# vressegu/sdeflow-light

Hardware: AMD Instinct MI355X
Metric: score-matching train steps/sec (+ reverse-SDE sample steps/sec) (higher is better)
Workload: dtype f32

## Files before the change

sdeflow_light_amd/csrc/conv_kernels.hip:

```cpp
#include "common.h"
#include <type_traits>
#include <stdlib.h>

#define CONV_MAX_SRC 2

__device__ __forceinline__ f32x4 mfma16c(float a, float b, f32x4 c) {
  return __builtin_amdgcn_mfma_f32_16x16x4f32(a, b, c, 0, 0, 0);
}

struct ConvGeom {
  int N, Hi, Wi, Ho, Wo;
  int KH, KW, strideH, padH, strideW, padW;
  int mode;
  int ups;
};

struct ConvArgs {
  ConvGeom g;
  const float* src[CONV_MAX_SRC];
  int C[CONV_MAX_SRC];
  int koff[CONV_MAX_SRC];
  int nsrc;
  const float* Wp;
  int Cout, CoutP, Ktot;
  const float* bias;
  const float* samp_bias;
  int n_bias, n_samp;
  float* out;
  int accumulate;
  const float* residual;
  const float* in_scale;
  const float* in_shift;
  int in_act;
  unsigned short tapmask_in[16];
  unsigned short tapmask_out[8];
  float* cstat;
  int cs_S;
};

__device__ __forceinline__ float row16_sum(float v) {
  v += __builtin_bit_cast(float, __builtin_amdgcn_update_dpp(0, __builtin_bit_cast(int, v), 0xB1, 0xF, 0xF, false));
  v += __builtin_bit_cast(float, __builtin_amdgcn_update_dpp(0, __builtin_bit_cast(int, v), 0x4E, 0xF, 0xF, false));
  v += __builtin_bit_cast(float, __builtin_amdgcn_update_dpp(0, __builtin_bit_cast(int, v), 0x141, 0xF, 0xF, false));
  v += __builtin_bit_cast(float, __builtin_amdgcn_update_dpp(0, __builtin_bit_cast(int, v), 0x140, 0xF, 0xF, false));
  return v;
}
__device__ __forceinline__ void cstat_store(const ConvArgs& A, int n, int slot, int co, f32x4 s, f32x4 ss, int il) {
#pragma unroll
  for (int r = 0; r < 4; ++r) { s[r] = row16_sum(s[r]); ss[r] = row16_sum(ss[r]); }
  if (il == 0) {
    float* cp = A.cstat + (((size_t)n * A.cs_S + slot) * 2) * A.Cout + co;
    *reinterpret_cast<f32x4*>(cp) = s;
    *reinterpret_cast<f32x4*>(cp + A.Cout) = ss;
  }
}


__device__ __forceinline__ bool src_coord(const ConvGeom& g, int o, int k, int in_size_up, int stride, int pad, int& i) {
  int v;
  if (g.mode == 0) {
    v = o * stride + k - pad;
  } else {
    const int t = o + pad - k;
    if (t < 0) return false;
    if (stride == 2) { if (t & 1) return false; v = t >> 1; }
    else if (stride == 1) v = t;
    else { if (t % stride) return false; v = t / stride; }
  }
  if (v < 0 || v >= in_size_up) return false;
  i = g.ups ? (v >> 1) : v;
  return true;
}

template <int MT, int NT, bool FAST>
__global__ void __launch_bounds__(256) k_conv_gemm(ConvArgs A) {
  const int tid = threadIdx.x, w = tid >> 6, lane = tid & 63, il = lane & 15, q = lane >> 4;
  const ConvGeom g = A.g;
  const int HoWo = g.Ho * g.Wo;
  const int Mtot = g.N * HoWo;
  const int m0 = (blockIdx.x * 4 + w) * (NT * 16);
  if (m0 >= Mtot) return;
  const int co0 = blockIdx.y * (MT * 16);
  const int Hup = g.ups ? 2 * g.Hi : g.Hi, Wup = g.ups ? 2 * g.Wi : g.Wi;
// ... 712 lines not shown
        valid |= 1u << k;
      }
    }
    st[k] = v;
  }
#pragma unroll
  for (int k = 0; k < NST; ++k) {
    const int idx = tid + 256 * k;
    if (idx < n_items) {
      f32x4 v = st[k];
      if (A.in_scale && ((valid >> k) & 1u)) {
        v = v * ga + gb;
        if (A.in_act == 1) {
#pragma unroll
          for (int r = 0; r < 4; ++r) v[r] = v[r] * __builtin_amdgcn_rcpf(1.0f + __expf(-v[r]));
        }
      }
      *reinterpret_cast<f32x4*>(cs_lds + (idx >> 3) * CT_P + 4 * c4) = v;
    }
  }
  __syncthreads();
  const int py = tid >> 4, px = tid & 15;
  float acc[CO];
#pragma unroll
  for (int co = 0; co < CO; ++co) acc[co] = 0.f;
#pragma unroll
  for (int tap = 0; tap < 9; ++tap) {
    const float* xp = cs_lds + ((py + tap / 3) * HW + px + tap % 3) * CT_P;
    const float* wt = A.Wp + (size_t)tap * A.CoutP * A.Ktot;
#pragma unroll
    for (int q4 = 0; q4 < 8; ++q4) {
      const f32x4 xv = *reinterpret_cast<const f32x4*>(xp + 4 * q4);
#pragma unroll
      for (int co = 0; co < CO; ++co) {
        const float* w = wt + (size_t)co * A.Ktot + 4 * q4;
        acc[co] = __builtin_fmaf(xv[0], w[0], acc[co]); acc[co] = __builtin_fmaf(xv[1], w[1], acc[co]);
        acc[co] = __builtin_fmaf(xv[2], w[2], acc[co]); acc[co] = __builtin_fmaf(xv[3], w[3], acc[co]);
      }
    }
#pragma unroll
    for (int co = 0; co < CO; ++co) asm volatile("" : "+v"(acc[co]));
  }
  const int oy = y0 + py, ox = x0 + px;
  if (oy < g.Ho && ox < g.Wo) {
    const size_t m = ((size_t)n * g.Ho + oy) * g.Wo + ox;
    float* op = A.out + m * CO;
#pragma unroll
    for (int co = 0; co < CO; ++co) {
      float v = acc[co];
      if (n < A.n_bias && A.bias) v += A.bias[co];
      if (A.samp_bias && n < A.n_samp) v += A.samp_bias[(size_t)n * CO + co];
      if (A.accumulate) v += op[co];
      if (A.residual) v += A.residual[m * CO + co];
      op[co] = v;
    }
  }
}

__device__ __forceinline__ float dpp_from_next_lane(float v) {
  return __builtin_bit_cast(float, __builtin_amdgcn_update_dpp(0, __builtin_bit_cast(int, v), 0x101 , 0xf, 0xf, true));
}
template <int HW_>
__device__ __forceinline__ void wino_patch_load(f32x4 (&d)[4][4], const float* __restrict__ p00, bool last_in_row) {
#pragma unroll
  for (int i = 0; i < 4; ++i) {
    d[i][0] = *reinterpret_cast<const f32x4*>(p00 + (i * HW_ + 0) * CT_P);
    d[i][1] = *reinterpret_cast<const f32x4*>(p00 + (i * HW_ + 1) * CT_P);
  }
#pragma unroll
  for (int i = 0; i < 4; ++i)
#pragma unroll
    for (int j = 0; j < 2; ++j)
#pragma unroll
      for (int r = 0; r < 4; ++r) d[i][2 + j][r] = dpp_from_next_lane(d[i][j][r]);
  if (last_in_row) {
#pragma unroll
    for (int i = 0; i < 4; ++i) {
      d[i][2] = *reinterpret_cast<const f32x4*>(p00 + (i * HW_ + 2) * CT_P);
      d[i][3] = *reinterpret_cast<const f32x4*>(p00 + (i * HW_ + 3) * CT_P);
    }
  }
}

template <int NCO, bool WL = false>
__global__ void __launch_bounds__(256, 2) k_conv_wino(ConvArgs A, int tiles_x, int tiles_y, int n_tiles, int n_cob, int n_tgrp) {
  extern __shared__ __attribute__((aligned(16))) float cw_lds[];
  const int tid = threadIdx.x, w = tid >> 6, lane = tid & 63, il = lane & 15, q = lane >> 4;
  const ConvGeom g = A.g;
  constexpr int HW = 18, halo = 18 * 18;
  float* cur = cw_lds;
  const int xcd = blockIdx.x & 7, loc = blockIdx.x >> 3;
  const int cob = loc % n_cob, tile = (loc / n_cob) * 8 + xcd;
  (void)n_tgrp;
  if (tile >= n_tiles) return;
  const int co0 = cob * (NCO * 16);
  const int tt = 16 * w + il, ty = tt >> 3, tx = tt & 7;
  const int pbase = (2 * ty * HW + 2 * tx) * CT_P + 4 * q;
  f32x4 acc[16][NCO];
#pragma unroll
  for (int p = 0; p < 16; ++p)
#pragma unroll
    for (int c = 0; c < NCO; ++c) acc[p][c] = f32x4{0, 0, 0, 0};

  int nch[CONV_MAX_SRC];
#pragma unroll
  for (int s = 0; s < CONV_MAX_SRC; ++s) nch[s] = s < A.nsrc ? (A.C[s] + CT_KC - 1) / CT_KC : 0;
  constexpr int MAXST = (halo * (CT_KC / 4) + 255) / 256;
  constexpr int n_items = halo * (CT_KC / 4);
  const int up = g.ups ? 1 : 0;
  const int ctot_all = A.C[0] + (A.nsrc > 1 ? A.C[1] : 0);
  int n, y0, x0;
  { int t = tile; const int tx_i = t % tiles_x; t /= tiles_x; const int ty_i = t % tiles_y; n = t / tiles_y; y0 = ty_i * 16; x0 = tx_i * 16; }
  auto stage = [&](int s_, int c0) __attribute__((always_inline)) {
    const int C = A.C[s_];
    const float* base = A.src[s_] + (size_t)n * g.Hi * g.Wi * C;
    f32x4 ga = {1.f, 1.f, 1.f, 1.f}, gb = {0.f, 0.f, 0.f, 0.f};
    const int cq = c0 + 4 * (tid & 7);
    if (A.in_scale && cq < C) {
      const size_t o = (size_t)n * ctot_all + (s_ ? A.C[0] : 0) + cq;
      ga = *reinterpret_cast<const f32x4*>(A.in_scale + o);
      gb = *reinterpret_cast<const f32x4*>(A.in_shift + o);
    }
    f32x4 st[MAXST];
    unsigned valid = 0;
#pragma unroll
    for (int k = 0; k < MAXST; ++k) {
      const int idx = tid + 256 * k;
      f32x4 v = {0, 0, 0, 0};
      if (idx < n_items) {
        const int hp = idx >> 3, hy = hp / HW, hx = hp - hy * HW;
        const int iy = y0 + hy - 1, ix = x0 + hx - 1;
        const int c = c0 + 4 * (idx & 7);
        if (iy >= 0 && iy < (g.Hi << up) && ix >= 0 && ix < (g.Wi << up) && c < C) {
          v = *reinterpret_cast<const f32x4*>(base + ((size_t)(iy >> up) * g.Wi + (ix >> up)) * C + c);
          valid |= 1u << k;
        }
      }
      st[k] = v;
    }
    if (A.in_scale) {
#pragma unroll
      for (int k = 0; k < MAXST; ++k) {
        if ((valid >> k) & 1u) {
          f32x4 v = st[k] * ga + gb;
          if (A.in_act == 1) {
#pragma unroll
            for (int r = 0; r < 4; ++r) v[r] = v[r] * __builtin_amdgcn_rcpf(1.0f + __expf(-v[r]));
          }
          st[k] = v;
        }
      }
    }
#pragma unroll
    for (int k = 0; k < MAXST; ++k) {
      const int idx = tid + 256 * k;
      if (idx < n_items) *reinterpret_cast<f32x4*>(cur + (idx >> 3) * CT_P + 4 * (idx & 7)) = st[k];
    }
  };

  const size_t a_co_stride = (size_t)16 * A.Ktot, pos_stride = (size_t)A.CoutP * A.Ktot;
  if constexpr (WL) {
    static_assert(NCO == 2, "the LDS weight image is laid out for two output-channel tiles");
    float* wbuf = cw_lds + halo * CT_P;
    auto ngrp_of = [&](int s_, int c_) { const int rem = A.C[s_] - c_ * CT_KC; return rem >= CT_KC ? 2 : ((rem + 15) >> 4); };
    auto wfill = [&](int s_, int c_, int g_, int half, int b) __attribute__((always_inline)) {
      const float* src = A.Wp + (size_t)(co0 + il) * A.Ktot + A.koff[s_] + c_ * CT_KC + 16 * g_ + 4 * q + (size_t)(8 * half) * pos_stride;
// ... 28 lines not shown
#pragma unroll
          for (int j = 0; j < 4; ++j) {
            const f32x4 r0 = d[0][j] - d[2][j], r1 = d[1][j] + d[2][j], r2 = d[2][j] - d[1][j], r3 = d[1][j] - d[3][j];
            d[0][j] = r0; d[1][j] = r1; d[2][j] = r2; d[3][j] = r3;
          }
#pragma unroll
          for (int i = 0; i < 4; ++i) {
            const f32x4 c0_ = d[i][0] - d[i][2], c1_ = d[i][1] + d[i][2], c2_ = d[i][2] - d[i][1], c3_ = d[i][1] - d[i][3];
            d[i][0] = c0_; d[i][1] = c1_; d[i][2] = c2_; d[i][3] = c3_;
          }
        }
        const float* wb = wbuf + (step & 1) * 4096 + lane * 4;
        f32x4 a0 = *reinterpret_cast<const f32x4*>(wb), a1 = *reinterpret_cast<const f32x4*>(wb + 256);
#pragma unroll
        for (int pl = 0; pl < 8; ++pl) {
          const f32x4 x0 = a0, x1 = a1;
          if (pl < 7) {
            a0 = *reinterpret_cast<const f32x4*>(wb + (2 * pl + 2) * 256);
            a1 = *reinterpret_cast<const f32x4*>(wb + (2 * pl + 3) * 256);
          }
          const int pos = 8 * half + pl;
          const f32x4 b = d[pos >> 2][pos & 3];
#pragma unroll
          for (int r = 0; r < 4; ++r) {
            acc[pos][0] = mfma16c(x0[r], b[r], acc[pos][0]);
            acc[pos][1] = mfma16c(x1[r], b[r], acc[pos][1]);
          }
          __builtin_amdgcn_sched_barrier(0);
        }
        ++step;
      }
      if (!more) break;
      cs = ns; cc = nc; grp = ng;
    }
  } else
  for (int cs = 0; cs < A.nsrc; ++cs)
    for (int cc = 0; cc < (cs ? nch[1] : nch[0]); ++cc) {
      asm volatile("s_waitcnt lgkmcnt(0)\n\ts_barrier" ::: "memory");
      stage(cs, cc * CT_KC);
      asm volatile("s_waitcnt lgkmcnt(0)\n\ts_barrier" ::: "memory");
      const int C = A.C[cs], c0 = cc * CT_KC;
      const int ngrp = (C - c0 >= CT_KC) ? 2 : ((C - c0 + 15) >> 4);
      const float* wbase = A.Wp + (size_t)(co0 + il) * A.Ktot + A.koff[cs] + c0 + 4 * q;
      f32x4 an[NCO];
#pragma unroll
      for (int c = 0; c < NCO; ++c) an[c] = *reinterpret_cast<const f32x4*>(wbase + c * a_co_stride);
      const float* wq = wbase;
      for (int grp = 0; grp < ngrp; ++grp) {
        f32x4 d[4][4];
        wino_patch_load<HW>(d, cur + pbase + 16 * grp, tx == 7);
#pragma unroll
        for (int j = 0; j < 4; ++j) {
          const f32x4 r0 = d[0][j] - d[2][j], r1 = d[1][j] + d[2][j], r2 = d[2][j] - d[1][j], r3 = d[1][j] - d[3][j];
          d[0][j] = r0; d[1][j] = r1; d[2][j] = r2; d[3][j] = r3;
        }
#pragma unroll
        for (int i = 0; i < 4; ++i) {
          const f32x4 c0_ = d[i][0] - d[i][2], c1_ = d[i][1] + d[i][2], c2_ = d[i][2] - d[i][1], c3_ = d[i][1] - d[i][3];
          d[i][0] = c0_; d[i][1] = c1_; d[i][2] = c2_; d[i][3] = c3_;
        }
        __builtin_amdgcn_sched_barrier(0);
#pragma unroll
        for (int pos = 0; pos < 16; ++pos) {
          f32x4 a[NCO];
#pragma unroll
          for (int c = 0; c < NCO; ++c) a[c] = an[c];
          if (pos < 15) wq += pos_stride;
          else wq = wbase + 16 * (grp + 1);
          asm volatile("" : "+v"(wq));
          if (pos < 15 || grp + 1 < ngrp) {
#pragma unroll
            for (int c = 0; c < NCO; ++c) an[c] = *reinterpret_cast<const f32x4*>(wq + c * a_co_stride);
          }
          const f32x4 b = d[pos >> 2][pos & 3];
#pragma unroll
          for (int r = 0; r < 4; ++r)
#pragma unroll
            for (int c = 0; c < NCO; ++c) acc[pos][c] = mfma16c(a[c][r], b[r], acc[pos][c]);
          __builtin_amdgcn_sched_barrier(0);
        }
      }
    }

  const bool primal = n < A.n_bias;
  const bool vec = (A.Cout & 3) == 0;
#pragma unroll
  for (int c = 0; c < NCO; ++c) {
    const int co = co0 + 16 * c + 4 * q;
    if (co >= A.Cout) continue;
    const bool full = vec && (co + 3 < A.Cout);
    f32x4 add = {0.f, 0.f, 0.f, 0.f};
    if (primal && A.bias) {
      if (full) add = *reinterpret_cast<const f32x4*>(A.bias + co);
      else
#pragma unroll
        for (int r = 0; r < 4; ++r) if (co + r < A.Cout) add[r] = A.bias[co + r];
    }
    if (A.samp_bias && n < A.n_samp) {
      const float* sbp = A.samp_bias + (size_t)n * A.Cout + co;
      if (full) add += *reinterpret_cast<const f32x4*>(sbp);
      else
#pragma unroll
        for (int r = 0; r < 4; ++r) if (co + r < A.Cout) add[r] += sbp[r];
    }
    f32x4 t0[4], t1[4];
#pragma unroll
    for (int nu = 0; nu < 4; ++nu) {
      t0[nu] = acc[nu][c] + acc[4 + nu][c] + acc[8 + nu][c];
      t1[nu] = acc[4 + nu][c] - acc[8 + nu][c] - acc[12 + nu][c];
    }
    f32x4 Y[2][2];
    Y[0][0] = t0[0] + t0[1] + t0[2]; Y[0][1] = t0[1] - t0[2] - t0[3];
    Y[1][0] = t1[0] + t1[1] + t1[2]; Y[1][1] = t1[1] - t1[2] - t1[3];
    f32x4 cs = {0.f, 0.f, 0.f, 0.f}, css = {0.f, 0.f, 0.f, 0.f};
#pragma unroll
    for (int dy = 0; dy < 2; ++dy)
#pragma unroll
      for (int dx = 0; dx < 2; ++dx) {
        const int oy = y0 + 2 * ty + dy, ox = x0 + 2 * tx + dx;
        if (oy >= g.Ho || ox >= g.Wo) continue;
        const size_t m = ((size_t)n * g.Ho + oy) * g.Wo + ox;
        f32x4 v = Y[dy][dx] + add;
        float* op = A.out + m * A.Cout + co;
        if (full) {
          if (A.accumulate) v += *reinterpret_cast<const f32x4*>(op);
          if (A.residual) v += *reinterpret_cast<const f32x4*>(A.residual + (op - A.out));
          *reinterpret_cast<f32x4*>(op) = v;
          cs += v; css += v * v;
        } else {
#pragma unroll
          for (int r = 0; r < 4; ++r)
            if (co + r < A.Cout) op[r] = (A.accumulate ? op[r] + v[r] : v[r]) + (A.residual ? A.residual[(op - A.out) + r] : 0.f);
        }
      }
    if (A.cstat) cstat_store(A, n, (tile - n * tiles_x * tiles_y) * 4 + w, co, cs, css, il);
  }
}

__global__ void __launch_bounds__(256, 1) k_conv_wino_p32(ConvArgs A, int tiles_x, int tiles_y, int n_tiles) {
  extern __shared__ __attribute__((aligned(16))) float cw_lds[];
  constexpr int NCO = 2, HW = 18, halo = 18 * 18;
  const int tid = threadIdx.x, w = tid >> 6, lane = tid & 63, il = lane & 15, q = lane >> 4;
  const ConvGeom g = A.g;
  float* wbuf = cw_lds;
  float* hb0 = cw_lds + 2 * 16 * 2 * 256;
  float* hb1 = hb0 + halo * CT_P;
  const int tt = 16 * w + il, ty = tt >> 3, tx = tt & 7;
  const int pbase = (2 * ty * HW + 2 * tx) * CT_P + 4 * q;
  const size_t a_co_stride = (size_t)16 * A.Ktot, pos_stride = (size_t)A.CoutP * A.Ktot;
  int t = blockIdx.x;
  if (t >= n_tiles) return;
  {
    const float* src = A.Wp + (size_t)il * A.Ktot + 4 * q;
#pragma unroll
    for (int j = 0; j < 16; ++j) {
      const int pw = 16 * w + j, grp = pw >> 5, pos = (pw >> 1) & 15, c = pw & 1;
      __builtin_amdgcn_global_load_lds((const __attribute__((address_space(1))) void*)(src + (size_t)pos * pos_stride + c * a_co_stride + 16 * grp),
                                       (__attribute__((address_space(3))) void*)(wbuf + pw * 256), 16, 0, 0);
    }
  }
  constexpr int MAXST = (halo * (CT_KC / 4) + 255) / 256;
  constexpr int n_items = halo * (CT_KC / 4);
  const int up = g.ups ? 1 : 0;
  const int C = A.C[0];
  f32x4 st[MAXST];
  f32x4 ga = {1.f, 1.f, 1.f, 1.f}, gb = {0.f, 0.f, 0.f, 0.f};
  unsigned valid = 0;
  auto origin = [&](int tile, int& n, int& y0, int& x0) {
    const int tx_i = tile % tiles_x; tile /= tiles_x;
    const int ty_i = tile % tiles_y; n = tile / tiles_y; y0 = ty_i * 16; x0 = tx_i * 16;
  };
  auto stage_load = [&](int tile) __attribute__((always_inline)) {
    int n, y0, x0;
    origin(tile, n, y0, x0);
    const float* base = A.src[0] + (size_t)n * g.Hi * g.Wi * C;
    const int cq = 4 * (tid & 7);
    ga = f32x4{1.f, 1.f, 1.f, 1.f}; gb = f32x4{0.f, 0.f, 0.f, 0.f};
    if (A.in_scale && cq < C) {
      const size_t o = (size_t)n * C + cq;
      ga = *reinterpret_cast<const f32x4*>(A.in_scale + o);
      gb = *reinterpret_cast<const f32x4*>(A.in_shift + o);
    }
    valid = 0;
#pragma unroll
    for (int k = 0; k < MAXST; ++k) {
      const int idx = tid + 256 * k;
      f32x4 v = {0, 0, 0, 0};
      if (idx < n_items) {
        const int hp = idx >> 3, hy = hp / HW, hx = hp - hy * HW;
        const int iy = y0 + hy - 1, ix = x0 + hx - 1;
        const int c = 4 * (idx & 7);
        if (iy >= 0 && iy < (g.Hi << up) && ix >= 0 && ix < (g.Wi << up) && c < C) {
          v = *reinterpret_cast<const f32x4*>(base + ((size_t)(iy >> up) * g.Wi + (ix >> up)) * C + c);
          valid |= 1u << k;
        }
      }
      st[k] = v;
    }
  };
  auto stage_store = [&](float* buf) __attribute__((always_inline)) {
    if (A.in_scale) {
#pragma unroll
      for (int k = 0; k < MAXST; ++k) {
        if ((valid >> k) & 1u) {
          f32x4 v = st[k] * ga + gb;
          if (A.in_act == 1) {
#pragma unroll
            for (int r = 0; r < 4; ++r) v[r] = v[r] * __builtin_amdgcn_rcpf(1.0f + __expf(-v[r]));
          }
          st[k] = v;
        }
      }
    }
#pragma unroll
    for (int k = 0; k < MAXST; ++k) {
      const int idx = tid + 256 * k;
      if (idx < n_items) *reinterpret_cast<f32x4*>(buf + (idx >> 3) * CT_P + 4 * (idx & 7)) = st[k];
    }
  };
  stage_load(t);
  stage_store(hb0);
  asm volatile("s_waitcnt vmcnt(0) lgkmcnt(0)\n\ts_barrier" ::: "memory");
  float* cur = hb0;
  float* nxt = hb1;
  const int ngrp = (C + 15) >> 4;
  const bool vec = (A.Cout & 3) == 0;
  for (; t < n_tiles; t += gridDim.x) {
    const int tn = t + gridDim.x;
    const bool more = tn < n_tiles;
    if (more) stage_load(tn);
    f32x4 acc[16][NCO];
#pragma unroll
    for (int p = 0; p < 16; ++p)
#pragma unroll
      for (int c = 0; c < NCO; ++c) acc[p][c] = f32x4{0, 0, 0, 0};
    for (int grp = 0; grp < ngrp; ++grp) {
      f32x4 d[4][4];
#pragma unroll
      for (int i = 0; i < 4; ++i)
#pragma unroll
        for (int j = 0; j < 4; ++j) d[i][j] = *reinterpret_cast<const f32x4*>(cur + pbase + (i * HW + j) * CT_P + 16 * grp);
#pragma unroll
      for (int j = 0; j < 4; ++j) {
        const f32x4 r0 = d[0][j] - d[2][j], r1 = d[1][j] + d[2][j], r2 = d[2][j] - d[1][j], r3 = d[1][j] - d[3][j];
        d[0][j] = r0; d[1][j] = r1; d[2][j] = r2; d[3][j] = r3;
      }
#pragma unroll
      for (int i = 0; i < 4; ++i) {
        const f32x4 c0_ = d[i][0] - d[i][2], c1_ = d[i][1] + d[i][2], c2_ = d[i][2] - d[i][1], c3_ = d[i][1] - d[i][3];
        d[i][0] = c0_; d[i][1] = c1_; d[i][2] = c2_; d[i][3] = c3_;
      }
      const float* wb = wbuf + grp * (16 * 2 * 256) + lane * 4;
      f32x4 a0 = *reinterpret_cast<const f32x4*>(wb), a1 = *reinterpret_cast<const f32x4*>(wb + 256);
#pragma unroll
      for (int pos = 0; pos < 16; ++pos) {
        const f32x4 x0_ = a0, x1_ = a1;
        if (pos < 15) {
          a0 = *reinterpret_cast<const f32x4*>(wb + (2 * pos + 2) * 256);
          a1 = *reinterpret_cast<const f32x4*>(wb + (2 * pos + 3) * 256);
        }
        const f32x4 b = d[pos >> 2][pos & 3];
#pragma unroll
        for (int r = 0; r < 4; ++r) {
          acc[pos][0] = mfma16c(x0_[r], b[r], acc[pos][0]);
          acc[pos][1] = mfma16c(x1_[r], b[r], acc[pos][1]);
        }
        __builtin_amdgcn_sched_barrier(0);
      }
    }
    int n, y0, x0;
    origin(t, n, y0, x0);
    const bool primal = n < A.n_bias;
#pragma unroll
    for (int c = 0; c < NCO; ++c) {
      const int co = 16 * c + 4 * q;
      if (co >= A.Cout) continue;
      const bool full = vec && (co + 3 < A.Cout);
      f32x4 add = {0.f, 0.f, 0.f, 0.f};
      if (primal && A.bias) {
        if (full) add = *reinterpret_cast<const f32x4*>(A.bias + co);
        else
#pragma unroll
          for (int r = 0; r < 4; ++r) if (co + r < A.Cout) add[r] = A.bias[co + r];
      }
      if (A.samp_bias && n < A.n_samp) {
        const float* sbp = A.samp_bias + (size_t)n * A.Cout + co;
        if (full) add += *reinterpret_cast<const f32x4*>(sbp);
        else
#pragma unroll
          for (int r = 0; r < 4; ++r) if (co + r < A.Cout) add[r] += sbp[r];
      }
      f32x4 t0[4], t1[4];
#pragma unroll
      for (int nu = 0; nu < 4; ++nu) {
        t0[nu] = acc[nu][c] + acc[4 + nu][c] + acc[8 + nu][c];
        t1[nu] = acc[4 + nu][c] - acc[8 + nu][c] - acc[12 + nu][c];
      }
      f32x4 Y[2][2];
      Y[0][0] = t0[0] + t0[1] + t0[2]; Y[0][1] = t0[1] - t0[2] - t0[3];
      Y[1][0] = t1[0] + t1[1] + t1[2]; Y[1][1] = t1[1] - t1[2] - t1[3];
      f32x4 cs = {0.f, 0.f, 0.f, 0.f}, css = {0.f, 0.f, 0.f, 0.f};
#pragma unroll
      for (int dy = 0; dy < 2; ++dy)
#pragma unroll
        for (int dx = 0; dx < 2; ++dx) {
          const int oy = y0 + 2 * ty + dy, ox = x0 + 2 * tx + dx;
          if (oy >= g.Ho || ox >= g.Wo) continue;
          const size_t m = ((size_t)n * g.Ho + oy) * g.Wo + ox;
          f32x4 v = Y[dy][dx] + add;
          float* op = A.out + m * A.Cout + co;
          if (full) {
            if (A.accumulate) v += *reinterpret_cast<const f32x4*>(op);
            if (A.residual) v += *reinterpret_cast<const f32x4*>(A.residual + (op - A.out));
            *reinterpret_cast<f32x4*>(op) = v;
            cs += v; css += v * v;
          } else {
#pragma unroll
            for (int r = 0; r < 4; ++r)
              if (co + r < A.Cout) op[r] = (A.accumulate ? op[r] + v[r] : v[r]) + (A.residual ? A.residual[(op - A.out) + r] : 0.f);
          }
        }
      if (A.cstat) cstat_store(A, n, (t - n * tiles_x * tiles_y) * 4 + w, co, cs, css, il);
    }
    if (more) stage_store(nxt);
    asm volatile("s_waitcnt lgkmcnt(0)\n\ts_barrier" ::: "memory");
    float* sw = cur; cur = nxt; nxt = sw;
  }
}

__global__ void __launch_bounds__(256) k_wino_pack_batched(const msgm_pack_job_t* __restrict__ jobs) {
  const msgm_pack_job_t J = jobs[blockIdx.y];
  const int64_t tot = (int64_t)J.rows * J.ncols;
  for (int64_t e = blockIdx.x * (int64_t)blockDim.x + threadIdx.x; e < tot; e += (int64_t)gridDim.x * blockDim.x) {
    const int c = (int)(e % J.ncols), r = (int)(e / J.ncols);
    const float* w = J.W + r * J.sr + (J.col_off + c) * J.sc;
    float gk[3][3], h[4][3];
#pragma unroll
    for (int t = 0; t < 9; ++t) gk[t / 3][t % 3] = w[t * J.st];
#pragma unroll
    for (int j = 0; j < 3; ++j) {
      h[0][j] = gk[0][j];
      h[1][j] = 0.5f * (gk[0][j] + gk[1][j] + gk[2][j]);
      h[2][j] = 0.5f * (gk[0][j] - gk[1][j] + gk[2][j]);
      h[3][j] = gk[2][j];
    }
#pragma unroll
    for (int i = 0; i < 4; ++i) {
      const float u0 = h[i][0], u1 = 0.5f * (h[i][0] + h[i][1] + h[i][2]), u2 = 0.5f * (h[i][0] - h[i][1] + h[i][2]), u3 = h[i][2];
      float* p = J.Wp + ((int64_t)(4 * i) * J.rowsP + r) * J.Ktot + J.kp_off + c;
      const int64_t ps = (int64_t)J.rowsP * J.Ktot;
      p[0] = u0; p[ps] = u1; p[2 * ps] = u2; p[3 * ps] = u3;
    }
  }
}

struct WgradArgs {
  ConvGeom g;
  const float* gy;
  const float* src;
  int C, koff;
  float* dWp;
  int Cout, CoutP, Ktot;
  int chunk;
  float* dbias;
  int n_bias;
  unsigned short tm_c[16], tm_o[16];
  float* slab; long slab_stride;
};

template <int MT, int KT>
__global__ void __launch_bounds__(256) k_conv_wgrad(WgradArgs A) {
  __shared__ float red[4][MT * KT * 256];
  const int tid = threadIdx.x, w = tid >> 6, lane = tid & 63, il = lane & 15, q = lane >> 4;
  const ConvGeom g = A.g;
  const int HoWo = g.Ho * g.Wo;
  const int Mtot = g.N * HoWo;
  const int cblocks = (A.C + 16 * KT - 1) / (16 * KT);
  const int coblk = blockIdx.y / cblocks, cblk = blockIdx.y - coblk * cblocks;
  const int co0 = coblk * 16 * MT, c0 = cblk * 16 * KT;
  const int tap = blockIdx.z;
  const int kh = tap / g.KW, kw = tap - kh * g.KW;
  const int Hup = g.ups ? 2 * g.Hi : g.Hi, Wup = g.ups ? 2 * g.Wi : g.Wi;
  const int mbeg = blockIdx.x * A.chunk;
  const int mend = min(mbeg + A.chunk, Mtot);

  f32x4 acc[MT][KT];
#pragma unroll
  for (int mt = 0; mt < MT; ++mt)
#pragma unroll
    for (int kt = 0; kt < KT; ++kt) acc[mt][kt] = f32x4{0, 0, 0, 0};

  int m = mbeg + 4 * w + q;
  int n = m / HoWo, oh, ow;
  { const int r = m - n * HoWo; oh = r / g.Wo; ow = r - oh * g.Wo; }
  const float* gyp[MT];
#pragma unroll
  for (int mt = 0; mt < MT; ++mt) gyp[mt] = A.gy + (size_t)m * A.Cout + co0 + 16 * mt + il;
  bool vco[MT], vc[KT];
#pragma unroll
  for (int mt = 0; mt < MT; ++mt) vco[mt] = co0 + 16 * mt + il < A.Cout;
#pragma unroll
  for (int kt = 0; kt < KT; ++kt) vc[kt] = c0 + 16 * kt + il < A.C;
  const size_t gy_step = (size_t)16 * A.Cout;
  for (int mg = mbeg + 4 * w; mg < mend; mg += 16) {
    const bool pin = m < mend;
    float a[MT], b[KT];
    int ih = 0, iw = 0;
    const bool ok = pin && src_coord(g, oh, kh, Hup, g.strideH, g.padH, ih) && src_coord(g, ow, kw, Wup, g.strideW, g.padW, iw);
#pragma unroll
// ... 670 lines not shown
  const int64_t tot = (int64_t)N * C;
  for (int64_t e = blockIdx.x * (int64_t)blockDim.x + threadIdx.x; e < tot; e += (int64_t)gridDim.x * blockDim.x) {
    const int n = (int)(e / C), c = (int)(e - (int64_t)n * C);
    out[e] = x[((size_t)n * P + pos) * C + c];
  }
}

static inline hipStream_t S(msgm_stream_t s) { return reinterpret_cast<hipStream_t>(s); }

static int check_geom(const msgm_conv_geom_t* g) {
  if (!g || g->N <= 0 || g->Hi <= 0 || g->Wi <= 0 || g->Ho <= 0 || g->Wo <= 0 || g->KH <= 0 || g->KW <= 0 ||
      g->strideH <= 0 || g->padH < 0 || g->strideW <= 0 || g->padW < 0 || (g->mode != 0 && g->mode != 1) ||
      (g->ups != 0 && g->ups != 1))
    return MSGM_E_BADARG;
  if ((int64_t)g->N * g->Ho * g->Wo >= (1ll << 31) || (int64_t)g->N * g->Hi * g->Wi >= (1ll << 31)) return MSGM_E_UNSUPPORTED;
  return MSGM_OK;
}
static ConvGeom to_geom(const msgm_conv_geom_t* g) {
  return ConvGeom{g->N, g->Hi, g->Wi, g->Ho, g->Wo, g->KH, g->KW, g->strideH, g->padH, g->strideW, g->padW, g->mode, g->ups};
}

extern "C" {

static bool conv_tile_eligible(const msgm_conv_geom_t* geom, int32_t C0, const float* src1, int32_t C1, int32_t CoutP) {
  const bool fast = (C0 % 16 == 0) && (!src1 || C1 % 16 == 0);
  const int ups_sh = geom->ups ? 1 : 0;
  const bool same = geom->strideH == 1 && geom->strideW == 1 && (!geom->ups || geom->mode == 0) &&
                    (geom->Hi << ups_sh) == geom->Ho && (geom->Wi << ups_sh) == geom->Wo &&
                    (geom->KH & 1) && (geom->KW & 1) && geom->padH == (geom->KH - 1) / 2 && geom->padW == (geom->KW - 1) / 2 &&
                    geom->KH <= 3 && geom->KW <= 3;
  return same && fast && CoutP % 32 == 0 && (int64_t)geom->Ho * geom->Wo >= 64 &&
         (geom->Ho > 1 ? geom->KH == geom->KW : geom->KH == 1) &&
         !getenv("MSGM_NO_CONV_TILE");
}

int msgm_conv_input_transform_supported(const msgm_conv_geom_t* geom, int32_t C0, int32_t C1, int32_t CoutP) {
  if (check_geom(geom)) return 0;
  static const float dummy = 0.f;
  return conv_tile_eligible(geom, C0, C1 > 0 ? &dummy : nullptr, C1, CoutP) ? 1 : 0;
}

static bool conv_wino_eligible(const msgm_conv_geom_t* geom, int32_t C0, int32_t C1, int32_t CoutP) {
  const int ups_sh = geom->ups ? 1 : 0;
  return geom->mode == 0 && geom->KH == 3 && geom->KW == 3 && geom->strideH == 1 && geom->strideW == 1 && geom->padH == 1 &&
         geom->padW == 1 && (geom->Hi << ups_sh) == geom->Ho && (geom->Wi << ups_sh) == geom->Wo && geom->Ho % 16 == 0 &&
         geom->Wo % 16 == 0 && C0 % 16 == 0 && C1 % 16 == 0 && CoutP % 32 == 0;
}

int msgm_conv_wino_supported(const msgm_conv_geom_t* geom, int32_t C0, int32_t C1, int32_t CoutP) {
  if (check_geom(geom)) return 0;
  return conv_wino_eligible(geom, C0, C1, CoutP) ? 1 : 0;
}

int msgm_wino_pack_weights_batched(const msgm_pack_job_t* jobs, int32_t n_jobs, msgm_stream_t stream) {
  if (!jobs || n_jobs <= 0) return MSGM_E_BADARG;
  hipLaunchKernelGGL(k_wino_pack_batched, dim3(8, (unsigned)n_jobs), dim3(256), 0, S(stream), jobs);
  return msgm_check_launch();
}

int msgm_conv_forward_wino(const msgm_conv_geom_t* geom, const float* src0, int32_t C0, const float* src1, int32_t C1,
                           const float* WpW, int32_t Cout, int32_t CoutP, int32_t Ktot, const float* bias,
                           const float* samp_bias, int32_t n_bias, int32_t n_samp, float* out, int32_t accumulate,
                           const msgm_conv_fuse_t* fuse, msgm_stream_t stream) {
  int rc = check_geom(geom);
  if (rc) return rc;
  if (fuse && ((fuse->in_scale == nullptr) != (fuse->in_shift == nullptr) || (fuse->in_act != 0 && fuse->in_act != 1)))
    return MSGM_E_BADARG;
  if (!src0 || !WpW || !out || C0 <= 0 || Cout <= 0 || (src1 && C1 <= 0)) return MSGM_E_BADARG;
  if (!conv_wino_eligible(geom, C0, src1 ? C1 : 0, CoutP)) return MSGM_E_UNSUPPORTED;
  const int k0 = ((C0 + 15) / 16) * 16, k1 = src1 ? ((C1 + 15) / 16) * 16 : 0;
  if (Ktot != k0 + k1 || CoutP < Cout) return MSGM_E_BADARG;
  ConvArgs A{};
  A.g = to_geom(geom);
  A.src[0] = src0; A.C[0] = C0; A.koff[0] = 0;
  A.src[1] = src1; A.C[1] = src1 ? C1 : 0; A.koff[1] = k0;
  A.nsrc = src1 ? 2 : 1;
  A.Wp = WpW; A.Cout = Cout; A.CoutP = CoutP; A.Ktot = Ktot;
  A.bias = bias; A.samp_bias = samp_bias; A.n_bias = n_bias; A.n_samp = n_samp; A.out = out; A.accumulate = accumulate;
  if (fuse && fuse->chanstats && (Cout & 3)) return MSGM_E_UNSUPPORTED;
  if (fuse) { A.residual = fuse->residual; A.in_scale = fuse->in_scale; A.in_shift = fuse->in_shift; A.in_act = fuse->in_act; }
  const int tiles_x = geom->Wo / 16, tiles_y = geom->Ho / 16;
  if (fuse && fuse->chanstats) { A.cstat = fuse->chanstats; A.cs_S = tiles_x * tiles_y * 4; }
  const int n_tiles = tiles_x * tiles_y * geom->N, gy = CoutP / 32;
  const size_t lds = (size_t)18 * 18 * CT_P * sizeof(float);
  dim3 grid((unsigned)(8 * gy * ((n_tiles + 7) / 8)));
  static const bool reg_weights = getenv("MSGM_WINO_REGW") != nullptr;
  static const bool no_p32 = getenv("MSGM_WINO_NO_P32") != nullptr;
  static const int p32_min = getenv("MSGM_WINO_P32_MIN") ? atoi(getenv("MSGM_WINO_P32_MIN")) : 1024;
  if (!reg_weights && !no_p32 && !src1 && Ktot == 32 && CoutP == 32 && n_tiles >= p32_min) {
    static const int once32 = [] {
      (void)hipFuncSetAttribute(reinterpret_cast<const void*>(&k_conv_wino_p32), hipFuncAttributeMaxDynamicSharedMemorySize, 160 * 1024);
      return 0;
    }();
    (void)once32;
    static const int n_cu = [] { int d = 0, n = 256; (void)hipGetDevice(&d); (void)hipDeviceGetAttribute(&n, hipDeviceAttributeMultiprocessorCount, d); return n > 0 ? n : 256; }();
    const size_t lds32 = ((size_t)2 * 16 * 2 * 256 + 2 * 18 * 18 * CT_P) * sizeof(float);
    hipLaunchKernelGGL(k_conv_wino_p32, dim3((unsigned)n_cu), dim3(256), lds32, S(stream), A, tiles_x, tiles_y, n_tiles);
    return msgm_check_launch();
  }
  if (reg_weights || Ktot < 64) {
    hipLaunchKernelGGL((k_conv_wino<2, false>), grid, dim3(256), lds, S(stream), A, tiles_x, tiles_y, n_tiles, gy, n_tiles);
    return msgm_check_launch();
  }
  static const int once = [] {
    (void)hipFuncSetAttribute(reinterpret_cast<const void*>(&k_conv_wino<2, true>), hipFuncAttributeMaxDynamicSharedMemorySize, 160 * 1024);
    return 0;
  }();
  (void)once;
  hipLaunchKernelGGL((k_conv_wino<2, true>), grid, dim3(256), lds + 2 * 4096 * sizeof(float), S(stream), A, tiles_x, tiles_y, n_tiles, gy, n_tiles);
  return msgm_check_launch();
}

__global__ void __launch_bounds__(256) k_b6_split(const float* __restrict__ Wp, __bf16* __restrict__ Wb, long n) {
  for (long e = (long)blockIdx.x * 256 + threadIdx.x; e < n; e += (long)gridDim.x * 256) {
    const float x = Wp[e];
    const __bf16 h = (__bf16)x;
    const float r1 = x - (float)h;
    const __bf16 m = (__bf16)r1;
    Wb[e] = h; Wb[n + e] = m; Wb[2 * n + e] = (__bf16)(r1 - (float)m);
  }
}

static bool conv_b6_eligible(const msgm_conv_geom_t* geom, int32_t C0, int32_t C1, int32_t CoutP) {
  const int ups_sh = geom->ups ? 1 : 0;
  return geom->mode == 0 && geom->KH == 3 && geom->KW == 3 && geom->strideH == 1 && geom->strideW == 1 && geom->padH == 1 &&
         geom->padW == 1 && (geom->Hi << ups_sh) == geom->Ho && (geom->Wi << ups_sh) == geom->Wo && geom->Ho % 16 == 0 && geom->Wo % 16 == 0 &&
         C0 % 32 == 0 && C1 % 32 == 0 && CoutP % 32 == 0;
}

int msgm_conv_b6_supported(const msgm_conv_geom_t* geom, int32_t C0, int32_t C1, int32_t CoutP) {
  if (check_geom(geom)) return 0;
  return conv_b6_eligible(geom, C0, C1, CoutP) ? 1 : 0;
}

int msgm_b6_split_weights(const float* Wp, void* Wb, int64_t n_elem, msgm_stream_t stream) {
  if (!Wp || !Wb || n_elem <= 0) return MSGM_E_BADARG;
  hipLaunchKernelGGL(k_b6_split, dim3((unsigned)grid_for(n_elem, 256, 2048)), dim3(256), 0, S(stream), Wp, static_cast<__bf16*>(Wb), (long)n_elem);
  return msgm_check_launch();
}

int msgm_conv_forward_b6(const msgm_conv_geom_t* geom, const float* src0, int32_t C0, const float* src1, int32_t C1,
                         const void* Wb, int32_t Cout, int32_t CoutP, int32_t Ktot, const float* bias,
                         const float* samp_bias, int32_t n_bias, int32_t n_samp, float* out, int32_t accumulate,
                         const msgm_conv_fuse_t* fuse, msgm_stream_t stream) {
  int rc = check_geom(geom);
  if (rc) return rc;
  if (fuse && ((fuse->in_scale == nullptr) != (fuse->in_shift == nullptr) || (fuse->in_act != 0 && fuse->in_act != 1)))
    return MSGM_E_BADARG;
  if (!src0 || !Wb || !out || C0 <= 0 || Cout <= 0 || (src1 && C1 <= 0)) return MSGM_E_BADARG;
  if (!conv_b6_eligible(geom, C0, src1 ? C1 : 0, CoutP)) return MSGM_E_UNSUPPORTED;
  if (Ktot != C0 + (src1 ? C1 : 0) || CoutP < Cout) return MSGM_E_BADARG;
  if (fuse)
    for (int i = 0; i < 16; ++i)
      if (fuse->tapmask_in[i] || (i < 8 && fuse->tapmask_out[i])) return MSGM_E_UNSUPPORTED;
  ConvArgs A{};
  A.g = to_geom(geom);
  A.src[0] = src0; A.C[0] = C0; A.koff[0] = 0;
  A.src[1] = src1; A.C[1] = src1 ? C1 : 0; A.koff[1] = C0;
  A.nsrc = src1 ? 2 : 1;
  A.Wp = static_cast<const float*>(Wb); A.Cout = Cout; A.CoutP = CoutP; A.Ktot = Ktot;
  A.bias = bias; A.samp_bias = samp_bias; A.n_bias = n_bias; A.n_samp = n_samp; A.out = out; A.accumulate = accumulate;
  if (fuse) { A.residual = fuse->residual; A.in_scale = fuse->in_scale; A.in_shift = fuse->in_shift; A.in_act = fuse->in_act; }
  const int nco = (CoutP % 64 == 0) ? 4 : 2;
  const int tiles_x = (geom->Wo + 15) / 16, tiles_y = (geom->Ho + 15) / 16;
  if (fuse && fuse->chanstats) {
    if (Cout & 3) return MSGM_E_UNSUPPORTED;
    A.cstat = fuse->chanstats; A.cs_S = tiles_x * tiles_y * 4;
  }
  const int n_tiles = tiles_x * tiles_y * geom->N, gy = CoutP / (16 * nco);
  int per = (int)(((int64_t)n_tiles * gy) / (512 * 8));
  if (per > 4) per = 4;
  if (per < 1) per = 1;
  const int n_tgrp = (n_tiles + per - 1) / per;
  dim3 grid((unsigned)(8 * gy * ((n_tgrp + 7) / 8)));
  const size_t lds = (size_t)18 * 18 * 52 * sizeof(float);
  static const int once = [] {
    (void)hipFuncSetAttribute(reinterpret_cast<const void*>(&k_conv_tile<16, 16, 4, 3, 4, false, true>), hipFuncAttributeMaxDynamicSharedMemorySize, 160 * 1024);
    (void)hipFuncSetAttribute(reinterpret_cast<const void*>(&k_conv_tile<16, 16, 2, 3, 4, false, true>), hipFuncAttributeMaxDynamicSharedMemorySize, 160 * 1024);
// ... 579 lines not shown
```

Before: 8.772.

## Add persistent pipelined Winograd conv kernel with async global-to-LDS prefetch

Adds a persistent Winograd F(2,3) conv kernel that streams weights and input halo tiles into double-buffered LDS with global_load_lds, prefetching the next channel group or tile while the current one runs MFMAs. It is used for every Winograd conv without a fused input scale, in place of the earlier per-tile kernels. The shared epilogue is moved into a helper. The aim is to hide global-load latency and cut launch and occupancy waste. The risks are a hand-tuned vmcnt wait count, XOR swizzle correctness, and padding reads redirected to a zero buffer.

```diff
diff --git a/sdeflow_light_amd/csrc/conv_kernels.hip b/sdeflow_light_amd/csrc/conv_kernels.hip
--- a/sdeflow_light_amd/csrc/conv_kernels.hip
+++ b/sdeflow_light_amd/csrc/conv_kernels.hip
@@ -1,4 +1,5 @@
 #include "common.h"
+#include <algorithm>
 #include <type_traits>
 #include <stdlib.h>
 
@@ -877,6 +878,66 @@
   }
 }
 
+template <int NCO>
+__device__ __forceinline__ void wino_epilogue(const ConvArgs& A, const f32x4 (&acc)[16][NCO], int n, int y0, int x0, int ty, int tx,
+                                              int co0, int slot, int lane) {
+  const ConvGeom g = A.g;
+  const int il = lane & 15, q = lane >> 4;
+  const bool primal = n < A.n_bias;
+  const bool vec = (A.Cout & 3) == 0;
+#pragma unroll
+  for (int c = 0; c < NCO; ++c) {
+    const int co = co0 + 16 * c + 4 * q;
+    if (co >= A.Cout) continue;
+    const bool full = vec && (co + 3 < A.Cout);
+    f32x4 add = {0.f, 0.f, 0.f, 0.f};
+    if (primal && A.bias) {
+      if (full) add = *reinterpret_cast<const f32x4*>(A.bias + co);
+      else
+#pragma unroll
+        for (int r = 0; r < 4; ++r) if (co + r < A.Cout) add[r] = A.bias[co + r];
+    }
+    if (A.samp_bias && n < A.n_samp) {
+      const float* sbp = A.samp_bias + (size_t)n * A.Cout + co;
+      if (full) add += *reinterpret_cast<const f32x4*>(sbp);
+      else
+#pragma unroll
+        for (int r = 0; r < 4; ++r) if (co + r < A.Cout) add[r] += sbp[r];
+    }
+    f32x4 t0[4], t1[4];
+#pragma unroll
+    for (int nu = 0; nu < 4; ++nu) {
+      t0[nu] = acc[nu][c] + acc[4 + nu][c] + acc[8 + nu][c];
+      t1[nu] = acc[4 + nu][c] - acc[8 + nu][c] - acc[12 + nu][c];
+    }
+    f32x4 Y[2][2];
+    Y[0][0] = t0[0] + t0[1] + t0[2]; Y[0][1] = t0[1] - t0[2] - t0[3];
+    Y[1][0] = t1[0] + t1[1] + t1[2]; Y[1][1] = t1[1] - t1[2] - t1[3];
+    f32x4 cs = {0.f, 0.f, 0.f, 0.f}, css = {0.f, 0.f, 0.f, 0.f};
+#pragma unroll
+    for (int dy = 0; dy < 2; ++dy)
+#pragma unroll
+      for (int dx = 0; dx < 2; ++dx) {
+        const int oy = y0 + 2 * ty + dy, ox = x0 + 2 * tx + dx;
+        if (oy >= g.Ho || ox >= g.Wo) continue;
+        const size_t m = ((size_t)n * g.Ho + oy) * g.Wo + ox;
+        f32x4 v = Y[dy][dx] + add;
+        float* op = A.out + m * A.Cout + co;
+        if (full) {
+          if (A.accumulate) v += *reinterpret_cast<const f32x4*>(op);
+          if (A.residual) v += *reinterpret_cast<const f32x4*>(A.residual + (op - A.out));
+          *reinterpret_cast<f32x4*>(op) = v;
+          cs += v; css += v * v;
+        } else {
+#pragma unroll
+          for (int r = 0; r < 4; ++r)
+            if (co + r < A.Cout) op[r] = (A.accumulate ? op[r] + v[r] : v[r]) + (A.residual ? A.residual[(op - A.out) + r] : 0.f);
+        }
+      }
+    if (A.cstat) cstat_store(A, n, slot, co, cs, css, il);
+  }
+}
+
 template <int NCO, bool WL = false>
 __global__ void __launch_bounds__(256, 2) k_conv_wino(ConvArgs A, int tiles_x, int tiles_y, int n_tiles, int n_cob, int n_tgrp) {
   extern __shared__ __attribute__((aligned(16))) float cw_lds[];
@@ -1071,59 +1132,7 @@
       }
     }
 
-  const bool primal = n < A.n_bias;
-  const bool vec = (A.Cout & 3) == 0;
-#pragma unroll
-  for (int c = 0; c < NCO; ++c) {
-    const int co = co0 + 16 * c + 4 * q;
-    if (co >= A.Cout) continue;
-    const bool full = vec && (co + 3 < A.Cout);
-    f32x4 add = {0.f, 0.f, 0.f, 0.f};
-    if (primal && A.bias) {
-      if (full) add = *reinterpret_cast<const f32x4*>(A.bias + co);
-      else
-#pragma unroll
-        for (int r = 0; r < 4; ++r) if (co + r < A.Cout) add[r] = A.bias[co + r];
-    }
-    if (A.samp_bias && n < A.n_samp) {
-      const float* sbp = A.samp_bias + (size_t)n * A.Cout + co;
-      if (full) add += *reinterpret_cast<const f32x4*>(sbp);
-      else
-#pragma unroll
-        for (int r = 0; r < 4; ++r) if (co + r < A.Cout) add[r] += sbp[r];
-    }
-    f32x4 t0[4], t1[4];
-#pragma unroll
-    for (int nu = 0; nu < 4; ++nu) {
-      t0[nu] = acc[nu][c] + acc[4 + nu][c] + acc[8 + nu][c];
-      t1[nu] = acc[4 + nu][c] - acc[8 + nu][c] - acc[12 + nu][c];
-    }
-    f32x4 Y[2][2];
-    Y[0][0] = t0[0] + t0[1] + t0[2]; Y[0][1] = t0[1] - t0[2] - t0[3];
-    Y[1][0] = t1[0] + t1[1] + t1[2]; Y[1][1] = t1[1] - t1[2] - t1[3];
-    f32x4 cs = {0.f, 0.f, 0.f, 0.f}, css = {0.f, 0.f, 0.f, 0.f};
-#pragma unroll
-    for (int dy = 0; dy < 2; ++dy)
-#pragma unroll
-      for (int dx = 0; dx < 2; ++dx) {
-        const int oy = y0 + 2 * ty + dy, ox = x0 + 2 * tx + dx;
-        if (oy >= g.Ho || ox >= g.Wo) continue;
-        const size_t m = ((size_t)n * g.Ho + oy) * g.Wo + ox;
-        f32x4 v = Y[dy][dx] + add;
-        float* op = A.out + m * A.Cout + co;
-        if (full) {
-          if (A.accumulate) v += *reinterpret_cast<const f32x4*>(op);
-          if (A.residual) v += *reinterpret_cast<const f32x4*>(A.residual + (op - A.out));
-          *reinterpret_cast<f32x4*>(op) = v;
-          cs += v; css += v * v;
-        } else {
-#pragma unroll
-          for (int r = 0; r < 4; ++r)
-            if (co + r < A.Cout) op[r] = (A.accumulate ? op[r] + v[r] : v[r]) + (A.residual ? A.residual[(op - A.out) + r] : 0.f);
-        }
-      }
-    if (A.cstat) cstat_store(A, n, (tile - n * tiles_x * tiles_y) * 4 + w, co, cs, css, il);
-  }
+  wino_epilogue<NCO>(A, acc, n, y0, x0, ty, tx, co0, (tile - n * tiles_x * tiles_y) * 4 + w, lane);
 }
 
 __global__ void __launch_bounds__(256, 1) k_conv_wino_p32(ConvArgs A, int tiles_x, int tiles_y, int n_tiles) {
@@ -1213,7 +1222,6 @@
   float* cur = hb0;
   float* nxt = hb1;
   const int ngrp = (C + 15) >> 4;
-  const bool vec = (A.Cout & 3) == 0;
   for (; t < n_tiles; t += gridDim.x) {
     const int tn = t + gridDim.x;
     const bool more = tn < n_tiles;
@@ -1259,61 +1267,154 @@
     }
     int n, y0, x0;
     origin(t, n, y0, x0);
-    const bool primal = n < A.n_bias;
-#pragma unroll
-    for (int c = 0; c < NCO; ++c) {
-      const int co = 16 * c + 4 * q;
-      if (co >= A.Cout) continue;
-      const bool full = vec && (co + 3 < A.Cout);
-      f32x4 add = {0.f, 0.f, 0.f, 0.f};
-      if (primal && A.bias) {
-        if (full) add = *reinterpret_cast<const f32x4*>(A.bias + co);
-        else
-#pragma unroll
-          for (int r = 0; r < 4; ++r) if (co + r < A.Cout) add[r] = A.bias[co + r];
-      }
-      if (A.samp_bias && n < A.n_samp) {
-        const float* sbp = A.samp_bias + (size_t)n * A.Cout + co;
-        if (full) add += *reinterpret_cast<const f32x4*>(sbp);
-        else
-#pragma unroll
-          for (int r = 0; r < 4; ++r) if (co + r < A.Cout) add[r] += sbp[r];
-      }
-      f32x4 t0[4], t1[4];
-#pragma unroll
-      for (int nu = 0; nu < 4; ++nu) {
-        t0[nu] = acc[nu][c] + acc[4 + nu][c] + acc[8 + nu][c];
-        t1[nu] = acc[4 + nu][c] - acc[8 + nu][c] - acc[12 + nu][c];
-      }
-      f32x4 Y[2][2];
-      Y[0][0] = t0[0] + t0[1] + t0[2]; Y[0][1] = t0[1] - t0[2] - t0[3];
-      Y[1][0] = t1[0] + t1[1] + t1[2]; Y[1][1] = t1[1] - t1[2] - t1[3];
-      f32x4 cs = {0.f, 0.f, 0.f, 0.f}, css = {0.f, 0.f, 0.f, 0.f};
-#pragma unroll
-      for (int dy = 0; dy < 2; ++dy)
-#pragma unroll
-        for (int dx = 0; dx < 2; ++dx) {
-          const int oy = y0 + 2 * ty + dy, ox = x0 + 2 * tx + dx;
-          if (oy >= g.Ho || ox >= g.Wo) continue;
-          const size_t m = ((size_t)n * g.Ho + oy) * g.Wo + ox;
-          f32x4 v = Y[dy][dx] + add;
-          float* op = A.out + m * A.Cout + co;
-          if (full) {
-            if (A.accumulate) v += *reinterpret_cast<const f32x4*>(op);
-            if (A.residual) v += *reinterpret_cast<const f32x4*>(A.residual + (op - A.out));
-            *reinterpret_cast<f32x4*>(op) = v;
-            cs += v; css += v * v;
-          } else {
-#pragma unroll
-            for (int r = 0; r < 4; ++r)
-              if (co + r < A.Cout) op[r] = (A.accumulate ? op[r] + v[r] : v[r]) + (A.residual ? A.residual[(op - A.out) + r] : 0.f);
-          }
-        }
-      if (A.cstat) cstat_store(A, n, (t - n * tiles_x * tiles_y) * 4 + w, co, cs, css, il);
-    }
+    wino_epilogue<NCO>(A, acc, n, y0, x0, ty, tx, 0, (t - n * tiles_x * tiles_y) * 4 + w, lane);
     if (more) stage_store(nxt);
     asm volatile("s_waitcnt lgkmcnt(0)\n\ts_barrier" ::: "memory");
     float* sw = cur; cur = nxt; nxt = sw;
+  }
+}
+
+constexpr int WP_HPIECES = 21;
+constexpr int WP_HSTAGE = WP_HPIECES * 64 * 4;
+constexpr int WP_LDS_BYTES = (2 * 4096 + 2 * WP_HSTAGE) * (int)sizeof(float);
+__device__ __attribute__((aligned(16))) float g_wino_zero[4];
+
+__global__ void __launch_bounds__(256, 2) k_conv_wino_pipe(ConvArgs A, int tiles_x, int tiles_y, int n_tiles, int n_cob) {
+  extern __shared__ __attribute__((aligned(16))) float cw_lds[];
+  constexpr int NCO = 2, HW = 18;
+  const int tid = threadIdx.x, lane = tid & 63, il = lane & 15, q = lane >> 4;
+  const int w = __builtin_amdgcn_readfirstlane(tid >> 6);
+  const ConvGeom g = A.g;
+  float* wbuf = cw_lds;
+  float* hbuf = cw_lds + 2 * 4096;
+  const int xcd = blockIdx.x & 7, loc_stride = gridDim.x >> 3;
+  int loc = blockIdx.x >> 3;
+  int tile = (loc / n_cob) * 8 + xcd, cob = loc % n_cob;
+  if (tile >= n_tiles) return;
+  const int ngrp = A.Ktot >> 4, tpi = tiles_x * tiles_y, up = g.ups ? 1 : 0;
+  const size_t a_co_stride = (size_t)16 * A.Ktot, pos_stride = (size_t)A.CoutP * A.Ktot;
+  const int tt = 16 * w + il, ty = tt >> 3, tx = tt & 7;
+  const int P0 = 2 * ty * HW + 2 * tx, h0 = (P0 >> 1) & 3;
+
+  auto wfill = [&](int cob_, int grp_, int half) __attribute__((always_inline)) {
+    const float* src = A.Wp + (size_t)(cob_ * (NCO * 16) + il) * A.Ktot + 16 * grp_ + 4 * q + (size_t)(8 * half) * pos_stride;
+#pragma unroll
+    for (int j = 0; j < 4; ++j) {
+      const int pw = 4 * w + j;
+      __builtin_amdgcn_global_load_lds((const __attribute__((address_space(1))) void*)(src + (size_t)(pw >> 1) * pos_stride + (pw & 1) * a_co_stride),
+                                       (__attribute__((address_space(3))) void*)(wbuf + half * 4096 + pw * 256), 16, 0, 0);
+    }
+  };
+  const int Hu = g.Hi << up, Wu = g.Wi << up;
+  auto hfill = [&](int tile_, int grp_, int b) __attribute__((always_inline)) {
+    const int n = tile_ / tpi, r = tile_ - n * tpi, ty_i = r / tiles_x, y0 = ty_i * 16, x0 = (r - ty_i * tiles_x) * 16;
+    const bool s1 = 16 * grp_ >= A.C[0];
+    const int C = s1 ? A.C[1] : A.C[0];
+    const float* base = (s1 ? A.src[1] : A.src[0]) + (size_t)n * g.Hi * g.Wi * C + (16 * grp_ - (s1 ? A.C[0] : 0));
+#pragma unroll
+    for (int j = 0; j < (WP_HPIECES + 3) / 4; ++j) {
+      const int m = w + 4 * j;
+      if (m < WP_HPIECES) {
+        const int sl = 64 * m + lane, P = sl >> 2, c = (sl & 3) ^ ((P >> 1) & 3);
+        const int hy = P / HW, hx = P - hy * HW, iy = y0 + hy - 1, ix = x0 + hx - 1;
+        const bool in = P < HW * HW && (unsigned)iy < (unsigned)Hu && (unsigned)ix < (unsigned)Wu;
+        const float* p = in ? base + (((iy >> up) * g.Wi + (ix >> up)) * C + 4 * c) : g_wino_zero;
+        __builtin_amdgcn_global_load_lds((const __attribute__((address_space(1))) void*)p,
+                                         (__attribute__((address_space(3))) void*)(hbuf + b * WP_HSTAGE + m * 256), 16, 0, 0);
+      }
+    }
+  };
+
+  f32x4 acc[16][NCO];
+#pragma unroll
+  for (int p = 0; p < 16; ++p)
+#pragma unroll
+    for (int c = 0; c < NCO; ++c) acc[p][c] = f32x4{0, 0, 0, 0};
+  int grp = 0, hb = 0;
+  wfill(cob, 0, 0);
+  hfill(tile, 0, 0);
+  for (;;) {
+    int nloc = loc, ntile = tile, ncob = cob, ngrp_ = grp + 1;
+    if (ngrp_ == ngrp) {
+      ngrp_ = 0; nloc = loc + loc_stride;
+      ntile = (nloc / n_cob) * 8 + xcd; ncob = nloc % n_cob;
+    }
+    const bool more = ntile < n_tiles;
+    f32x4 d[4][4];
+#pragma unroll
+    for (int half = 0; half < 2; ++half) {
+      if (half == 1 && more) asm volatile("s_waitcnt vmcnt(5) lgkmcnt(0)\n\ts_barrier" ::: "memory");
+      else asm volatile("s_waitcnt vmcnt(0) lgkmcnt(0)\n\ts_barrier" ::: "memory");
+      if (half == 0) {
+        wfill(cob, grp, 1);
+        if (more) hfill(ntile, ngrp_, hb ^ 1);
+      } else if (more) {
+        wfill(ncob, ngrp_, 0);
+      }
+      if (half == 0) {
+        const float* hs = hbuf + hb * WP_HSTAGE;
+#pragma unroll
+        for (int i = 0; i < 4; ++i) {
+          const float* rp = hs + 16 * (P0 + i * HW) + 4 * (q ^ ((h0 + i) & 3));
+          d[i][0] = *reinterpret_cast<const f32x4*>(rp);
+          d[i][1] = *reinterpret_cast<const f32x4*>(rp + 16);
+        }
+#pragma unroll
+        for (int i = 0; i < 4; ++i)
+#pragma unroll
+          for (int j = 0; j < 2; ++j)
+#pragma unroll
+            for (int r = 0; r < 4; ++r) d[i][2 + j][r] = dpp_from_next_lane(d[i][j][r]);
+        if (tx == 7) {
+#pragma unroll
+          for (int i = 0; i < 4; ++i) {
+            const float* rp = hs + 16 * (P0 + i * HW + 2) + 4 * (q ^ ((h0 + i + 1) & 3));
+            d[i][2] = *reinterpret_cast<const f32x4*>(rp);
+            d[i][3] = *reinterpret_cast<const f32x4*>(rp + 16);
+          }
+        }
+#pragma unroll
+        for (int j = 0; j < 4; ++j) {
+          const f32x4 r0 = d[0][j] - d[2][j], r1 = d[1][j] + d[2][j], r2 = d[2][j] - d[1][j], r3 = d[1][j] - d[3][j];
+          d[0][j] = r0; d[1][j] = r1; d[2][j] = r2; d[3][j] = r3;
+        }
+#pragma unroll
+        for (int i = 0; i < 4; ++i) {
+          const f32x4 c0_ = d[i][0] - d[i][2], c1_ = d[i][1] + d[i][2], c2_ = d[i][2] - d[i][1], c3_ = d[i][1] - d[i][3];
+          d[i][0] = c0_; d[i][1] = c1_; d[i][2] = c2_; d[i][3] = c3_;
+        }
+      }
+      const float* wb = wbuf + half * 4096 + lane * 4;
+      f32x4 a0 = *reinterpret_cast<const f32x4*>(wb), a1 = *reinterpret_cast<const f32x4*>(wb + 256);
+#pragma unroll
+      for (int pl = 0; pl < 8; ++pl) {
+        const f32x4 x0_ = a0, x1_ = a1;
+        if (pl < 7) {
+          a0 = *reinterpret_cast<const f32x4*>(wb + (2 * pl + 2) * 256);
+          a1 = *reinterpret_cast<const f32x4*>(wb + (2 * pl + 3) * 256);
+        }
+        const int pos = 8 * half + pl;
+        const f32x4 b = d[pos >> 2][pos & 3];
+#pragma unroll
+        for (int r = 0; r < 4; ++r) {
+          acc[pos][0] = mfma16c(x0_[r], b[r], acc[pos][0]);
+          acc[pos][1] = mfma16c(x1_[r], b[r], acc[pos][1]);
+        }
+        __builtin_amdgcn_sched_barrier(0);
+      }
+    }
+    if (ngrp_ == 0) {
+      asm volatile("s_nop 15\n\ts_nop 7" ::: "memory");
+      __builtin_amdgcn_sched_barrier(0);
+      const int n = tile / tpi, r = tile - n * tpi, ty_i = r / tiles_x;
+      wino_epilogue<NCO>(A, acc, n, ty_i * 16, (r - ty_i * tiles_x) * 16, ty, tx, cob * (NCO * 16), r * 4 + w, lane);
+      if (!more) break;
+#pragma unroll
+      for (int p = 0; p < 16; ++p)
+#pragma unroll
+        for (int c = 0; c < NCO; ++c) acc[p][c] = f32x4{0, 0, 0, 0};
+    }
+    loc = nloc; tile = ntile; cob = ncob; grp = ngrp_; hb ^= 1;
   }
 }
 
@@ -2150,6 +2251,18 @@
   const int tiles_x = geom->Wo / 16, tiles_y = geom->Ho / 16;
   if (fuse && fuse->chanstats) { A.cstat = fuse->chanstats; A.cs_S = tiles_x * tiles_y * 4; }
   const int n_tiles = tiles_x * tiles_y * geom->N, gy = CoutP / 32;
+  static const int n_cu = [] { int d = 0, n = 256; (void)hipGetDevice(&d); (void)hipDeviceGetAttribute(&n, hipDeviceAttributeMultiprocessorCount, d); return n > 0 ? n : 256; }();
+  if (!A.in_scale) {
+    static const int once_pipe = [] {
+      (void)hipFuncSetAttribute(reinterpret_cast<const void*>(&k_conv_wino_pipe), hipFuncAttributeMaxDynamicSharedMemorySize, WP_LDS_BYTES);
+      return 0;
+    }();
+    (void)once_pipe;
+    const int items_per_xcd = gy * ((n_tiles + 7) / 8);
+    const int wg_per_xcd = std::min(items_per_xcd, std::max(1, 2 * n_cu / 8));
+    hipLaunchKernelGGL(k_conv_wino_pipe, dim3((unsigned)(8 * wg_per_xcd)), dim3(256), WP_LDS_BYTES, S(stream), A, tiles_x, tiles_y, n_tiles, gy);
+    return msgm_check_launch();
+  }
   const size_t lds = (size_t)18 * 18 * CT_P * sizeof(float);
   dim3 grid((unsigned)(8 * gy * ((n_tiles + 7) / 8)));
   static const bool reg_weights = getenv("MSGM_WINO_REGW") != nullptr;
@@ -2161,7 +2274,6 @@
       return 0;
     }();
     (void)once32;
-    static const int n_cu = [] { int d = 0, n = 256; (void)hipGetDevice(&d); (void)hipDeviceGetAttribute(&n, hipDeviceAttributeMultiprocessorCount, d); return n > 0 ? n : 256; }();
     const size_t lds32 = ((size_t)2 * 16 * 2 * 256 + 2 * 18 * 18 * CT_P) * sizeof(float);
     hipLaunchKernelGGL(k_conv_wino_p32, dim3((unsigned)n_cu), dim3(256), lds32, S(stream), A, tiles_x, tiles_y, n_tiles);
     return msgm_check_launch();
```

New measurement: 9.336, median of 6. 6.4% higher.
